# ToKe79/nuts333

Hardware: AMD Instinct MI355X
Metric: delivered_broadcast_lines_per_s (higher is better)
Workload: dtype u8

## Files before the change

### nuts333_amd/device/fanout.hip

```cpp

#include <hip/hip_runtime.h>
#include <hipcub/hipcub.hpp>

#include <algorithm>
#include <chrono>
#include <cstdint>
#include <cstdio>
#include <cstring>

namespace {

constexpr int kOutBuff = 1000;
constexpr int kTextSize = 2000;
constexpr int kNumCols = 21;
constexpr int kMaxWrites = 16;
constexpr int kBlock = 256;

constexpr uint8_t kLogin = 1, kHasRoom = 2, kSameRoom = 4, kIgnall = 8, kIgnshout = 16, kSender = 32, kColour = 64;
constexpr int kComShout = 4, kComSemote = 7;

__constant__ char kColCom[kNumCols][2] = {
    {'R', 'S'}, {'O', 'L'}, {'U', 'L'}, {'L', 'I'}, {'R', 'V'}, {'F', 'K'}, {'F', 'R'}, {'F', 'G'}, {'F', 'Y'}, {'F', 'B'},
    {'F', 'M'}, {'F', 'T'}, {'F', 'W'}, {'B', 'K'}, {'B', 'R'}, {'B', 'G'}, {'B', 'Y'}, {'B', 'B'}, {'B', 'M'}, {'B', 'T'},
    {'B', 'W'},
// ... 79 lines not shown
        } else if (ch == '~') {
            if (k.pos > kOutBuff - 6) k.flush();
            const int c = colcom_at(s, i, len);
            if (c >= 0) {
                if (colour) {
                    k.put(27); k.put('['); k.put((uint8_t)kColArg[c][0]);
                    if (kColArg[c][1]) k.put((uint8_t)kColArg[c][1]);
                    k.put('m');
                }
                i += 3;
            } else {
                k.put('~');
                i++;
            }
        } else {
            k.put(ch);
            i++;
        }
        if (k.pos == kOutBuff) k.flush();
    }
    if (k.pos) k.flush();
    if (colour) {
        k.reset_code();
        k.flush();
    }
}

struct Args {
    const uint8_t* text;
    const int32_t* text_off;
    const int32_t* text_len;
    const uint8_t* rec;
    int n;
    int rm_is_null, force_listen, com_num;
    uint8_t* admitted;
    int64_t* nbytes;
    int32_t* nwrites;
    int64_t* out_off;
    int32_t* w_off;
    int* violations;
    uint8_t* arena;
    int64_t arena_cap;
    int32_t* wsz;
    int64_t wsz_cap;
};

template <bool BROADCAST>
__device__ __forceinline__ bool load_item(const Args& a, int i, const uint8_t*& s, int& len)
{
    if (BROADCAST) {
        __shared__ uint8_t lds[kTextSize];
        len = a.text_len[0];
        for (int j = threadIdx.x; j < len; j += blockDim.x) lds[j] = a.text[j];
        __syncthreads();
        s = lds;
        return i < a.n;
    }
    if (i >= a.n) return false;
    s = a.text + a.text_off[i];
    len = a.text_len[i];
    return true;
}

template <bool BROADCAST>
__device__ void measure(const Args& a)
{
    const int i = blockIdx.x * blockDim.x + threadIdx.x;
    if (i == 0) {
        a.nbytes[a.n] = 0;
        a.nwrites[a.n] = 0;
    }
    const uint8_t* s;
    int len;
    if (!load_item<BROADCAST>(a, i, s, len)) return;
    const uint8_t l = a.rec[i];
    const bool in = !BROADCAST || admits(l, a.rm_is_null, a.force_listen, a.com_num);
    Sink<false> k{nullptr, nullptr, 0, 0};
    if (in) transduce(s, len, (l & kColour) != 0, k);
    if (k.n > 6 * (int64_t)len + 4 || k.writes > kMaxWrites) atomicAdd(a.violations, 1);
    a.admitted[i] = in;
    a.nbytes[i] = k.n;
    a.nwrites[i] = k.writes;
}

template <bool BROADCAST>
__device__ void emit(const Args& a)
{
    const int i = blockIdx.x * blockDim.x + threadIdx.x;
    const uint8_t* s;
    int len;
    if (!load_item<BROADCAST>(a, i, s, len) || !a.admitted[i]) return;
    const int64_t room = a.arena_cap - a.out_off[i], wroom = a.wsz_cap - a.w_off[i];
    const int64_t cap = a.nbytes[i] < room ? a.nbytes[i] : (room > 0 ? room : 0);
    const int wcap = (int)(a.nwrites[i] < wroom ? a.nwrites[i] : (wroom > 0 ? wroom : 0));
    Sink<true> k{a.arena + a.out_off[i], a.wsz + a.w_off[i], cap, wcap};
    transduce(s, len, (a.rec[i] & kColour) != 0, k);
}

constexpr int kVarCap = 6 * (kTextSize - 1) + 4;
constexpr int kGroup = 16;

struct ManyArgs {
    const uint8_t* text;
    const int32_t* text_off;
    const int32_t* text_len;
    const uint8_t* flags;
    const int32_t* com_num;
    const int32_t* item_off;
    const int32_t* tile_off;
    const uint8_t* rec;
    int k, m;
    int* violations;
    uint8_t* admitted;
    int64_t* out_off;
    int32_t* w_off;
    int64_t* nbytes;
    int32_t* nwrites;
    uint8_t* arena;
    int64_t arena_cap;
    int32_t* wsz;
    int64_t wsz_cap;
};

struct Tile {
    int b, lo, hi;
};

__device__ __forceinline__ Tile find_tile(const ManyArgs& a)
{
// ... 238 lines not shown
            const int64_t off = a.out_off[i], woff = a.w_off[i];
            const int64_t room = a.arena_cap - off, wroom = a.wsz_cap - woff;
            int64_t n = in ? a.out_off[i + 1] - off : 0;
            n = n < room ? n : room;
            n = n < cap ? n : cap;
            int64_t nw = in ? a.w_off[i + 1] - woff : 0;
            nw = nw < wroom ? nw : wroom;
            nw = nw < kMaxWrites ? nw : kMaxWrites;
            s_off[threadIdx.x] = off;
            s_n[threadIdx.x] = n > 0 ? n : 0;
            s_woff[threadIdx.x] = (int32_t)woff;
            s_nw[threadIdx.x] = nw > 0 ? (int32_t)nw : 0;
            s_c[threadIdx.x] = (a.slot[j] & kColour) ? 1 : 0;
        }
    }
    const uint8_t* src = a.var + var_at(a.text_off[b], b);
    const int64_t stride = var_stride(len);
    for (int c = 0; c < 2; c++) {
        const int64_t n = a.vn[2 * b + c] < cap ? a.vn[2 * b + c] : cap;
        for (int64_t q = threadIdx.x; q < n; q += kBlock) var[c * kVarCap + q] = src[c * stride + q];
        const int nw = a.vw[2 * b + c] < kMaxWrites ? a.vw[2 * b + c] : kMaxWrites;
        if ((int)threadIdx.x < nw) vwsz[c * kMaxWrites + threadIdx.x] = a.vwsz[(2 * b + c) * kMaxWrites + threadIdx.x];
        if (threadIdx.x == 0) {
            vn[c] = n;
            vw[c] = nw;
        }
    }
    __syncthreads();
    const int count = a.capacity - j0 < kBlock ? a.capacity - j0 : kBlock;
    copy_items(count, var, vwsz, vn, vw, s_off, s_n, s_woff, s_nw, s_c, a.arena, a.wsz);
}

static_assert(2 * kMaxWrites <= kBlock, "roster kernels move a broadcast's chunk sizes with one lane each");

struct PlanArgs {
    const int32_t* room;
    const uint8_t* slot;
    const uint8_t* text;
    const int32_t* text_off;
    const int32_t* text_len;
    const int32_t* rm;
    const int32_t* sender;
    const uint8_t* flags;
    const int32_t* com_num;
    int k, capacity, tiles;
    int words;
    int* violations;
    int64_t* vn;
    int32_t* vw;
    int32_t* vwsz;
    uint64_t* bits;
    uint8_t* var;
};

__device__ void roster_plan(const PlanArgs& a)
{
    const int b = (int)blockIdx.x / a.tiles, tile = (int)blockIdx.x - b * a.tiles;
    const int j = tile * kBlock + (int)threadIdx.x;
    bool in = false;
    if (j < a.capacity) {
        const int rm = a.rm[b];
        const uint8_t l = listener_record(a.room[j], a.slot[j], rm, a.sender[b], j);
        in = admits(l, rm < 0, (a.flags[b] >> 1) & 1, a.com_num[b]);
    }
    const uint64_t word = __ballot(in);
    const int w = j >> 6;
// ... 2954 lines not shown
static_assert(64 * kReadSlice >= kArrSize && kWordLen + 7 <= 64, "roster_set: the word masks cover the longest inpstr, a lane per byte of word[1]");

struct SetOrderArgs {
    const int32_t* slot;
    const int32_t* rid;
    const uint8_t* com;
    int k;
    int8_t* outcome;
    int32_t* clen;

    static constexpr int kKeys = 4, kTexts = kSetTexts, kDeferred = kSetDeferred, kMapWords = 3 * kOrderSlotWords;
    __device__ void load(int b, bool live, int (&key)[kKeys]) const
    {
        key[0] = live ? slot[b] : 0, key[1] = live ? rid[b] : 0, key[2] = live && clen[b] >= 0, key[3] = live && com[b] == kComTopic;
    }
    static __device__ bool hit(const int (&key)[kKeys], const uint32_t* slots)
    {
        return bit_of(slots, key[0]) || (key[2] && bit_of(slots + kOrderSlotWords, key[1])) ||
               (key[3] && bit_of(slots + 2 * kOrderSlotWords, key[1]));
    }
    static __device__ void touch(const int (&key)[kKeys], int outcome, uint32_t* slots)
    {
        if (outcome > kSetIgntellOff) return;
        set_bit(slots, key[0]);
        if (outcome == kSetIgnallOn || outcome == kSetIgnallOff || outcome == kSetColourOn || outcome == kSetColourOff)
            set_bit(slots + kOrderSlotWords, key[1]);
        if (outcome == kSetTopicSet) set_bit(slots + 2 * kOrderSlotWords, key[1]);
    }
    __device__ void also_void(int) const {}
};

}

extern "C" __global__ void __launch_bounds__(kBlock) nuts_fanout_measure_batch(Args a) { measure<false>(a); }
extern "C" __global__ void __launch_bounds__(kBlock) nuts_fanout_measure_broadcast(Args a) { measure<true>(a); }
extern "C" __global__ void __launch_bounds__(kBlock) nuts_fanout_emit_batch(Args a) { emit<false>(a); }
extern "C" __global__ void __launch_bounds__(kBlock) nuts_fanout_emit_broadcast(Args a) { emit<true>(a); }
extern "C" __global__ void __launch_bounds__(kBlock) nuts_fanout_measure_many(ManyArgs a) { measure_many(a); }
extern "C" __global__ void __launch_bounds__(kBlock) nuts_fanout_emit_many(ManyArgs a) { emit_many(a); }
extern "C" __global__ void __launch_bounds__(kBlock) nuts_roster_measure(RosterArgs a) { roster_measure(a); }
extern "C" __global__ void __launch_bounds__(kBlock) nuts_roster_emit(RosterArgs a) { roster_emit(a); }
extern "C" __global__ void __launch_bounds__(kBlock) nuts_roster_plan(PlanArgs a) { roster_plan(a); }
extern "C" __global__ void __launch_bounds__(kBlock) nuts_roster_record(RecordArgs a) { roster_record<kRevLines>(a); }
extern "C" __global__ void __launch_bounds__(kBlock) nuts_roster_review(ReviewArgs a) { roster_review<kRevLines>(a); }
extern "C" __global__ void __launch_bounds__(kBlock) nuts_roster_speak(SpeakArgs a) { roster_speak(a); }
extern "C" __global__ void __launch_bounds__(kBlock) nuts_roster_speak_plan(SpeakPlanArgs a) { roster_speak_plan(a); }
extern "C" __global__ void __launch_bounds__(kBlock) nuts_roster_parse(ParseArgs a) { roster_parse(a); }
extern "C" __global__ void __launch_bounds__(kBlock) nuts_roster_tell(TellArgs a) { roster_tell(a); }
extern "C" __global__ void __launch_bounds__(kBlock) nuts_roster_record_tell(RecordArgs a) { roster_record<kTellLines>(a); }
extern "C" __global__ void __launch_bounds__(kBlock) nuts_roster_revtell(ReviewArgs a) { roster_review<kTellLines>(a); }
extern "C" __global__ void __launch_bounds__(kBlock) nuts_roster_look(LookArgs a) { roster_look(a); }
extern "C" __global__ void __launch_bounds__(kBlock) nuts_roster_relay(RelayArgs a) { roster_relay(a); }
extern "C" __global__ void __launch_bounds__(kBlock) nuts_roster_who(WhoArgs a) { roster_who(a); }
extern "C" __global__ void __launch_bounds__(kBlock) nuts_roster_who_shown(WhoArgs a) { roster_who_shown(a); }
extern "C" __global__ void __launch_bounds__(kBlock) nuts_roster_rooms_count(RoomsArgs a) { roster_rooms_count(a); }
extern "C" __global__ void __launch_bounds__(kBlock) nuts_roster_rooms_lines(RoomsArgs a) { roster_rooms_lines(a); }
extern "C" __global__ void __launch_bounds__(kBlock) nuts_roster_go(GoArgs a) { roster_go(a); }
extern "C" __global__ void __launch_bounds__(kBlock) nuts_roster_go_order(GoOrderArgs a) { order_events(a); }
extern "C" __global__ void __launch_bounds__(kBlock) nuts_roster_access(AccessArgs a) { roster_access(a); }
extern "C" __global__ void __launch_bounds__(kBlock) nuts_roster_access_order(AccessOrderArgs a) { order_events(a); }
extern "C" __global__ void __launch_bounds__(kBlock) nuts_roster_clone(CloneArgs a) { roster_clone(a); }
extern "C" __global__ void __launch_bounds__(kBlock) nuts_roster_clone_order(CloneOrderArgs a) { order_events(a); }
extern "C" __global__ void __launch_bounds__(kBlock) nuts_roster_set(SetArgs a) { roster_set(a); }
extern "C" __global__ void __launch_bounds__(kBlock) nuts_roster_set_order(SetOrderArgs a) { order_events(a); }


namespace {

struct Buffers {
    uint8_t* d_block = nullptr;
// ... 128 lines not shown
    if (timing) {
        timing->kernels_us = (double)ms * 1e3;
        timing->end_to_end_us = (t1 - t0) * 1e-3;
    }
    return 0;
}

template <typename T>
int fill_timing(T* timing, double t0, double t1, size_t h2d_bytes, size_t d2h_bytes)
{
    if (fill_timing(timing, t0, t1)) return -1;
    if (timing) {
        timing->h2d_bytes = (int64_t)h2d_bytes;
        timing->d2h_bytes = (int64_t)d2h_bytes;
    }
    return 0;
}

int check_bounds(int violations, const char* what)
{
    if (!violations) return 0;
    snprintf(g_err, sizeof(g_err), "%d %s(s) exceeded the hard output bounds (6*len+4 bytes, %d writes)", violations,
             what, kMaxWrites);
    return -1;
}

int fetch_results(const uint8_t* d, size_t res_at, size_t res_bytes)
{
    ND_CHECK(hipEventRecord(g.ev1, g.stream));
    ND_CHECK(hipMemcpyAsync(gm.res, d + res_at, res_bytes, hipMemcpyDeviceToHost, g.stream));
    ND_CHECK(hipStreamSynchronize(g.stream));
    return 0;
}

size_t layout_many(uintptr_t base, size_t text_bytes, size_t scan_bytes, ManyArgs& a, uint8_t** scan)
{
    Carver take{base};
    const size_t k = (size_t)a.k, m = (size_t)a.m;
    take(a.text, text_bytes);
    take(a.text_off, k);
    take(a.text_len, k);
    take(a.flags, k);
    take(a.com_num, k);
    take(a.item_off, k + 1);
    take(a.tile_off, k + 1);
    take(a.rec, m);
    take(a.violations, 1);
    take(a.admitted, m);
    take(a.out_off, m + 1);
    take(a.w_off, m + 1);
    take(a.nbytes, m + 1);
    take(a.nwrites, m + 1);
    take(a.arena, (size_t)a.arena_cap);
    take(a.wsz, (size_t)a.wsz_cap);
    take(*scan, scan_bytes);
    return take.at;
}

constexpr int kMaxRosters = 64;
constexpr int kMaxCapacity = 65536;

enum KeptId { kKeptSpeech, kKeptAfk, kKeptRooms, kKeptUdesc, kKeptWho, kKeptClones, kKeptNames, kKeptGo, kKeptCount };
struct KeptTable {
    const char* what;
    uint8_t* d = nullptr;
};

struct Roster {
    bool live = false;
    bool resident = false;
    int capacity = 0;
    int64_t rooms = 0;
    uint8_t* d = nullptr;
    uint8_t* mirror = nullptr;
    size_t cap_d = 0, cap_mirror = 0;
    int review_rooms = 0;
    uint8_t* rings = nullptr;
    bool revtell = false;
    uint8_t* tell_rings = nullptr;
    int look_rooms = 0;
    int clones = 0;
    KeptTable kept[kKeptCount] = {{"speaker table"}, {"AFK messages"}, {"room table"}, {"user descriptions"},
                                  {"who table"}, {"clone records"}, {"room names"}, {"go table"}};
};
Roster g_rosters[kMaxRosters];

void take_clones(Carver& take, int clones, const int32_t*& owner, const int32_t*& room, const uint8_t*& hear)
{
// ... 778 lines not shown
    return rocprim::make_transform_iterator(rocprim::make_counting_iterator(0),
                                            ItemCount<int32_t>{a.admitted, a.slot, a.vw, a.capacity, m});
}

Roster* roster_at(int handle)
{
    if (handle < 0 || handle >= kMaxRosters || !g_rosters[handle].live) {
        snprintf(g_err, sizeof(g_err), "no live roster %d", handle);
        return nullptr;
    }
    return &g_rosters[handle];
}

}

extern "C" {

struct nd_timing {
    double kernels_us;
    double end_to_end_us;
};

const char* nd_last_error(void) { return g_err; }

int nd_device_count(void)
{
    int n = 0;
    hipError_t e = hipGetDeviceCount(&n);
    if (e == hipErrorNoDevice) return 0;
    if (e != hipSuccess) return fail("hipGetDeviceCount", e);
    return n;
}

int nd_fanout(int broadcast, const uint8_t* text, int64_t text_bytes, const int32_t* text_off, const int32_t* text_len,
              const uint8_t* rec, int n, int rm_is_null, int force_listen, int com_num, uint8_t* admitted,
              int64_t* out_off, int32_t* w_off, nd_timing* timing)
{
    if (ensure_ready()) return -1;
    if (n < 1) {
        snprintf(g_err, sizeof(g_err), "empty batch");
        return -1;
    }
    const double t0 = now_ns();
    hipStream_t st = g.stream;
    Args a{};
    a.n = n;
    a.rm_is_null = rm_is_null;
    a.force_listen = force_listen;
    a.com_num = com_num;
    a.arena_cap = 4 * (int64_t)n + 6 * text_bytes * (broadcast ? n : 1);
    a.wsz_cap = (int64_t)n * kMaxWrites;
    size_t scan1 = 0, scan2 = 0;
    ND_CHECK(hipcub::DeviceScan::ExclusiveSum(nullptr, scan1, a.nbytes, a.out_off, n + 1, st));
    ND_CHECK(hipcub::DeviceScan::ExclusiveSum(nullptr, scan2, a.nwrites, a.w_off, n + 1, st));
    const size_t scan_bytes = std::max(scan1, scan2);
    uint8_t* scan = nullptr;
    const size_t need = layout(0, (size_t)text_bytes, scan_bytes, a, &scan);
    if (grow_dev(&g.d_block, &g.cap_block, need, "device buffers")) return -1;
    layout((uintptr_t)g.d_block, (size_t)text_bytes, scan_bytes, a, &scan);

    ND_CHECK(hipMemcpyAsync((void*)a.text, text, (size_t)text_bytes, hipMemcpyHostToDevice, st));
    ND_CHECK(hipMemcpyAsync((void*)a.text_len, text_len, (broadcast ? 1 : (size_t)n) * sizeof(int32_t), hipMemcpyHostToDevice, st));
    if (!broadcast) ND_CHECK(hipMemcpyAsync((void*)a.text_off, text_off, (size_t)n * sizeof(int32_t), hipMemcpyHostToDevice, st));
    ND_CHECK(hipMemcpyAsync((void*)a.rec, rec, (size_t)n, hipMemcpyHostToDevice, st));
    ND_CHECK(hipMemsetAsync(a.violations, 0, sizeof(int), st));

    const dim3 grid((unsigned)((n + kBlock - 1) / kBlock)), block(kBlock);
    ND_CHECK(hipEventRecord(g.ev0, st));
    hipLaunchKernelGGL(broadcast ? nuts_fanout_measure_broadcast : nuts_fanout_measure_batch, grid, block, 0, st, a);
    ND_CHECK(hipGetLastError());
    size_t bytes = scan_bytes;
    ND_CHECK(hipcub::DeviceScan::ExclusiveSum(scan, bytes, a.nbytes, a.out_off, n + 1, st));
    bytes = scan_bytes;
    ND_CHECK(hipcub::DeviceScan::ExclusiveSum(scan, bytes, a.nwrites, a.w_off, n + 1, st));
    hipLaunchKernelGGL(broadcast ? nuts_fanout_emit_broadcast : nuts_fanout_emit_batch, grid, block, 0, st, a);
    ND_CHECK(hipGetLastError());
    ND_CHECK(hipEventRecord(g.ev1, st));

    int violations = 0;
    ND_CHECK(hipMemcpyAsync(admitted, a.admitted, (size_t)n, hipMemcpyDeviceToHost, st));
    ND_CHECK(hipMemcpyAsync(out_off, a.out_off, ((size_t)n + 1) * sizeof(int64_t), hipMemcpyDeviceToHost, st));
    ND_CHECK(hipMemcpyAsync(w_off, a.w_off, ((size_t)n + 1) * sizeof(int32_t), hipMemcpyDeviceToHost, st));
    ND_CHECK(hipMemcpyAsync(&violations, a.violations, sizeof(int), hipMemcpyDeviceToHost, st));
    ND_CHECK(hipStreamSynchronize(st));
    if (check_bounds(violations, "item")) return -1;
    if (grow_host(&g.h_arena, &g.cap_host_arena, (size_t)out_off[n] + 1, "pinned arena")) return -1;
    if (grow_host(&g.h_wsz, &g.cap_host_writes, (size_t)w_off[n] + 1, "pinned write sizes")) return -1;
    ND_CHECK(hipMemcpyAsync(g.h_arena, a.arena, (size_t)out_off[n], hipMemcpyDeviceToHost, st));
    ND_CHECK(hipMemcpyAsync(g.h_wsz, a.wsz, (size_t)w_off[n] * sizeof(int32_t), hipMemcpyDeviceToHost, st));
    ND_CHECK(hipStreamSynchronize(st));
    const double t1 = now_ns();

    return fill_timing(timing, t0, t1);
}

const uint8_t* nd_arena(void) { return g.h_arena; }
const int32_t* nd_write_sizes(void) { return g.h_wsz; }

int nd_fanout_many(int k, const uint8_t* text, int64_t text_bytes, const int32_t* text_off, const int32_t* text_len,
                   const uint8_t* flags, const int32_t* com_num, const int32_t* item_off, const uint8_t* rec,
                   uint8_t* admitted, int64_t* out_off, int32_t* w_off, nd_timing* timing)
{
    if (ensure_ready()) return -1;
    if (k < 1 || item_off[0] != 0) {
        snprintf(g_err, sizeof(g_err), "empty call, or item offsets that do not start at 0");
        return -1;
    }
    for (int b = 0; b < k; b++)
// ... 1327 lines not shown
```

### nuts333_amd/devpath.py

```python
from __future__ import annotations

import argparse
import ctypes
import json
import statistics
import subprocess
import sys
import time
from pathlib import Path
from typing import NamedTuple

import numpy as np

from nuts333_amd import device, nuts_path

REPO = Path(__file__).resolve().parent.parent
PATHBENCH = REPO / "oracle" / "_build" / "pathbench"

TEXTS = {
    "say": b"Uaaa says: synthetic broadcast line 000123 from the nuts333 bench\n",
    "shout": b"~OLUaaa shouts:~RS synthetic broadcast line 000123 from the nuts333 bench\n",
}
COM = {"say": device.COM_SAY, "shout": device.COM_SHOUT}
SIZES = (10, 100, 1000)
# ... 1140 lines not shown
    if ngpu < 1:
        print("devpath: no GPU visible; this command measures the device path and has no CPU fall-back",
              file=sys.stderr)
        return 2

    t_start = time.perf_counter()
    pb = pathbench(a.pathbench_iterations)
    cases = []
    for n in SIZES:
        for text in TEXTS:
            for colour in COLOURS:
                table = listeners(n, colour)
                run = lambda: device.broadcast(TEXTS[text], table, 0, 0, COM[text])
                first = run()
                expect = sum(len(nuts_path.transduce(TEXTS[text], int(c))) for c in colours(n, colour)[1:])
                if int(first.out_offsets[-1]) != expect or int(first.admitted.sum()) != n - 1:
                    raise SystemExit(f"devpath: {n}/{text}/{colour}: device produced {int(first.out_offsets[-1])} "
                                     f"bytes, the CPU restatement {expect}")
                times = _timed(f"{n}/{text}/{colour}", {"broadcast": run}, a.reps, a.warmup)["broadcast"].times
                cpu = cpu_derived_us(pb, text, colour, n)
                cases.append({"n": n, "text": text, "colour": colour, "recipients": n - 1,
                              "bytes_out": int(first.out_offsets[-1]), "writes": int(first.write_offsets[-1]),
                              "kernels_us": times["kernels_us"], "end_to_end_us": times["end_to_end_us"],
                              "cpu_derived_us": round(cpu, 3),
                              "end_to_end_over_cpu": round(times["end_to_end_us"]["median"] / cpu, 1)})
    sections = {}
    for option, _, _, section in SECTIONS:
        counts = getattr(a, option.replace("-", "_"))
        if counts:
            sections.update(globals()[section](counts, a.reps, a.warmup, pb))
    out = {
        "what": "user-space stage of one broadcast (admit predicate + transducer), device vs CPU",
        "device": "gfx950",
        "kernels": ["nuts_fanout_measure_broadcast", "rocprim device scan x2", "nuts_fanout_emit_broadcast"],
        "reps": a.reps, "warmup": a.warmup,
        "end_to_end_covers": "listener table + text H2D, kernels, admitted/offsets/arena/write-size D2H, synchronise",
        "cpu_derived_from": {"pathbench": {k: v for k, v in pb.items() if k not in ("sink", "admitted")},
                             "formula": "(N-1) x transduce + N x fanout_predicate + format_line_once (derived, not timed)"},
        "cases": cases,
        **sections,
        "wall_s": round(time.perf_counter() - t_start, 1),
    }
    print(json.dumps(out))
    return 0


if __name__ == "__main__":
    sys.exit(main())
```

Before: 738,300.

## Broadcast fanout: transduce two colour variants once, place recipients by tile counts

The broadcast path no longer transduces the text once per recipient and runs two device scans. Instead it renders the coloured and plain variants once, counts admitted recipients per colour in each tile with ballots, and computes every output offset arithmetically from those counts. It also packs all inputs into one pinned H2D copy and copies results back in a head-sized D2H with a tail copy only when needed. This removes per-recipient transducer work, the scan launches, and several small transfers and syncs. In exchange the emit kernel serially sums the counts of all earlier tiles and uses more LDS.

```diff
diff --git a/nuts333_amd/device/fanout.hip b/nuts333_amd/device/fanout.hip
--- a/nuts333_amd/device/fanout.hip
+++ b/nuts333_amd/device/fanout.hip
@@ -135,7 +135,6 @@
     const int32_t* text_len;
     const uint8_t* rec;
     int n;
-    int rm_is_null, force_listen, com_num;
     uint8_t* admitted;
     int64_t* nbytes;
     int32_t* nwrites;
@@ -148,24 +147,14 @@
     int64_t wsz_cap;
 };
 
-template <bool BROADCAST>
 __device__ __forceinline__ bool load_item(const Args& a, int i, const uint8_t*& s, int& len)
 {
-    if (BROADCAST) {
-        __shared__ uint8_t lds[kTextSize];
-        len = a.text_len[0];
-        for (int j = threadIdx.x; j < len; j += blockDim.x) lds[j] = a.text[j];
-        __syncthreads();
-        s = lds;
-        return i < a.n;
-    }
     if (i >= a.n) return false;
     s = a.text + a.text_off[i];
     len = a.text_len[i];
     return true;
 }
 
-template <bool BROADCAST>
 __device__ void measure(const Args& a)
 {
     const int i = blockIdx.x * blockDim.x + threadIdx.x;
@@ -175,24 +164,22 @@
     }
     const uint8_t* s;
     int len;
-    if (!load_item<BROADCAST>(a, i, s, len)) return;
+    if (!load_item(a, i, s, len)) return;
     const uint8_t l = a.rec[i];
-    const bool in = !BROADCAST || admits(l, a.rm_is_null, a.force_listen, a.com_num);
     Sink<false> k{nullptr, nullptr, 0, 0};
-    if (in) transduce(s, len, (l & kColour) != 0, k);
+    transduce(s, len, (l & kColour) != 0, k);
     if (k.n > 6 * (int64_t)len + 4 || k.writes > kMaxWrites) atomicAdd(a.violations, 1);
-    a.admitted[i] = in;
+    a.admitted[i] = true;
     a.nbytes[i] = k.n;
     a.nwrites[i] = k.writes;
 }
 
-template <bool BROADCAST>
 __device__ void emit(const Args& a)
 {
     const int i = blockIdx.x * blockDim.x + threadIdx.x;
     const uint8_t* s;
     int len;
-    if (!load_item<BROADCAST>(a, i, s, len) || !a.admitted[i]) return;
+    if (!load_item(a, i, s, len) || !a.admitted[i]) return;
     const int64_t room = a.arena_cap - a.out_off[i], wroom = a.wsz_cap - a.w_off[i];
     const int64_t cap = a.nbytes[i] < room ? a.nbytes[i] : (room > 0 ? room : 0);
     const int wcap = (int)(a.nwrites[i] < wroom ? a.nwrites[i] : (wroom > 0 ? wroom : 0));
@@ -502,6 +489,144 @@
 }
 
 static_assert(2 * kMaxWrites <= kBlock, "roster kernels move a broadcast's chunk sizes with one lane each");
+
+struct BroadcastArgs {
+    const uint8_t* text;
+    const int32_t* text_off;
+    const int32_t* text_len;
+    const uint8_t* rec;
+    int n;
+    int rm_is_null, force_listen, com_num;
+    int* violations;
+    uint8_t* admitted;
+    int32_t* tile_cnt;
+    int64_t* out_off;
+    int32_t* w_off;
+    uint8_t* var;
+    int64_t* vn;
+    int32_t* vw;
+    int32_t* vwsz;
+    uint8_t* arena;
+    int64_t arena_cap;
+    int32_t* wsz;
+    int64_t wsz_cap;
+};
+
+constexpr int kWaves = kBlock / 64;
+
+__device__ __forceinline__ void count_tile(bool in, int c, int (*cnt)[kWaves], uint64_t* below)
+{
+    const uint64_t b0 = __ballot(in && c == 0), b1 = __ballot(in && c != 0);
+    const int wave = (int)threadIdx.x >> 6, lane = (int)threadIdx.x & 63;
+    if (lane == 0) {
+        cnt[0][wave] = __popcll(b0);
+        cnt[1][wave] = __popcll(b1);
+    }
+    const uint64_t lt = ((uint64_t)1 << lane) - 1;
+    below[0] = b0 & lt;
+    below[1] = b1 & lt;
+    __syncthreads();
+}
+
+__device__ void broadcast_measure(const BroadcastArgs& a)
+{
+    __shared__ int cnt[2][kWaves];
+    const int64_t i = (int64_t)blockIdx.x * kBlock + threadIdx.x;
+    bool in = false;
+    int c = 0;
+    if (i < a.n) {
+        const uint8_t l = a.rec[i];
+        in = admits(l, a.rm_is_null, a.force_listen, a.com_num);
+        c = (l & kColour) ? 1 : 0;
+        a.admitted[i] = in;
+    }
+    uint64_t below[2];
+    count_tile(in, c, cnt, below);
+    if (threadIdx.x < 2) {
+        int sum = 0;
+        for (int w = 0; w < kWaves; w++) sum += cnt[threadIdx.x][w];
+        a.tile_cnt[2 * (int64_t)blockIdx.x + threadIdx.x] = sum;
+    }
+    if (blockIdx.x == 0) store_variants(a, 0);
+}
+
+__device__ void broadcast_emit(const BroadcastArgs& a)
+{
+    __shared__ uint8_t var[2 * kVarCap];
+    __shared__ int32_t vwsz[2 * kMaxWrites];
+    __shared__ int64_t vn[2];
+    __shared__ int vw[2];
+    __shared__ int64_t s_off[kBlock], s_n[kBlock];
+    __shared__ int32_t s_woff[kBlock], s_nw[kBlock];
+    __shared__ uint8_t s_c[kBlock];
+    __shared__ int cnt[2][kWaves];
+    __shared__ int base[2];
+    const int64_t i0 = (int64_t)blockIdx.x * kBlock, i = i0 + threadIdx.x;
+    const int len = a.text_len[0];
+    const int64_t cap = 6 * (int64_t)len + 4;
+    if (threadIdx.x < 2) base[threadIdx.x] = 0;
+    bool in = false;
+    int c = 0;
+    if (i < a.n) {
+        in = a.admitted[i] != 0;
+        c = (a.rec[i] & kColour) ? 1 : 0;
+    }
+    uint64_t below[2];
+    count_tile(in, c, cnt, below);
+    {
+        int t0 = 0, t1 = 0;
+        for (int t = (int)threadIdx.x; t < (int)blockIdx.x; t += kBlock) {
+            t0 += a.tile_cnt[2 * (int64_t)t];
+            t1 += a.tile_cnt[2 * (int64_t)t + 1];
+        }
+        if (t0) atomicAdd(&base[0], t0);
+        if (t1) atomicAdd(&base[1], t1);
+    }
+    const int64_t stride = var_stride(len);
+    for (int v = 0; v < 2; v++) {
+        const int64_t n = a.vn[v] < cap ? a.vn[v] : cap;
+        for (int64_t q = threadIdx.x; q < n; q += kBlock) var[v * kVarCap + q] = a.var[v * stride + q];
+        const int nw = a.vw[v] < kMaxWrites ? a.vw[v] : kMaxWrites;
+        if ((int)threadIdx.x < nw) vwsz[v * kMaxWrites + threadIdx.x] = a.vwsz[v * kMaxWrites + threadIdx.x];
+        if (threadIdx.x == 0) {
+            vn[v] = n;
+            vw[v] = nw;
+        }
+    }
+    __syncthreads();
+    if (i < a.n) {
+        const int wave = (int)threadIdx.x >> 6;
+        int64_t e0 = base[0] + __popcll(below[0]), e1 = base[1] + __popcll(below[1]);
+        for (int w = 0; w < wave; w++) {
+            e0 += cnt[0][w];
+            e1 += cnt[1][w];
+        }
+        const int64_t off = e0 * a.vn[0] + e1 * a.vn[1];
+        const int64_t woff = e0 * (int64_t)a.vw[0] + e1 * (int64_t)a.vw[1];
+        const int64_t mine = in ? a.vn[c] : 0, wmine = in ? a.vw[c] : 0;
+        a.out_off[i] = off;
+        a.w_off[i] = (int32_t)woff;
+        if (i == a.n - 1) {
+            a.out_off[a.n] = off + mine;
+            a.w_off[a.n] = (int32_t)(woff + wmine);
+        }
+        const int64_t room = a.arena_cap - off, wroom = a.wsz_cap - woff;
+        int64_t n = mine < room ? mine : room;
+        n = n < cap ? n : cap;
+        int64_t nw = wmine < wroom ? wmine : wroom;
+        nw = nw < kMaxWrites ? nw : kMaxWrites;
+        s_off[threadIdx.x] = off;
+        s_n[threadIdx.x] = n > 0 ? n : 0;
+        s_woff[threadIdx.x] = (int32_t)woff;
+        s_nw[threadIdx.x] = nw > 0 ? (int32_t)nw : 0;
+        s_c[threadIdx.x] = (uint8_t)c;
+    }
+    __syncthreads();
+    const int64_t left = a.n - i0;
+    copy_items(left < kBlock ? (int)left : kBlock, var, vwsz, vn, vw, s_off, s_n, s_woff, s_nw, s_c, a.arena, a.wsz);
+}
+
+static_assert(kWaves >= 1 && kBlock >= 2, "the broadcast kernels: whole waves, and a lane per colour");
 
 struct PlanArgs {
     const int32_t* room;
@@ -3522,10 +3647,10 @@
 
 }
 
-extern "C" __global__ void __launch_bounds__(kBlock) nuts_fanout_measure_batch(Args a) { measure<false>(a); }
-extern "C" __global__ void __launch_bounds__(kBlock) nuts_fanout_measure_broadcast(Args a) { measure<true>(a); }
-extern "C" __global__ void __launch_bounds__(kBlock) nuts_fanout_emit_batch(Args a) { emit<false>(a); }
-extern "C" __global__ void __launch_bounds__(kBlock) nuts_fanout_emit_broadcast(Args a) { emit<true>(a); }
+extern "C" __global__ void __launch_bounds__(kBlock) nuts_fanout_measure_batch(Args a) { measure(a); }
+extern "C" __global__ void __launch_bounds__(kBlock) nuts_fanout_measure_broadcast(BroadcastArgs a) { broadcast_measure(a); }
+extern "C" __global__ void __launch_bounds__(kBlock) nuts_fanout_emit_batch(Args a) { emit(a); }
+extern "C" __global__ void __launch_bounds__(kBlock) nuts_fanout_emit_broadcast(BroadcastArgs a) { broadcast_emit(a); }
 extern "C" __global__ void __launch_bounds__(kBlock) nuts_fanout_measure_many(ManyArgs a) { measure_many(a); }
 extern "C" __global__ void __launch_bounds__(kBlock) nuts_fanout_emit_many(ManyArgs a) { emit_many(a); }
 extern "C" __global__ void __launch_bounds__(kBlock) nuts_roster_measure(RosterArgs a) { roster_measure(a); }
@@ -3720,6 +3845,31 @@
     ND_CHECK(hipStreamSynchronize(g.stream));
     return 0;
 }
+
+size_t layout_broadcast(uintptr_t base, size_t text_bytes, BroadcastArgs& a)
+{
+    Carver take{base};
+    const size_t n = (size_t)a.n, tiles = (n + kBlock - 1) / kBlock;
+    take(a.text, text_bytes);
+    take(a.text_off, 1);
+    take(a.text_len, 1);
+    take(a.rec, n);
+    take(a.violations, 1);
+    take(a.vn, 2);
+    take(a.vw, 2);
+    take(a.admitted, n);
+    take(a.out_off, n + 1);
+    take(a.w_off, n + 1);
+    take(a.wsz, (size_t)a.wsz_cap);
+    take(a.arena, (size_t)a.arena_cap);
+    take(a.tile_cnt, 2 * tiles);
+    take(a.vwsz, 2 * kMaxWrites);
+    take(a.var, (size_t)(2 * var_stride((int)text_bytes)));
+    return take.at;
+}
+
+constexpr int64_t kArenaHeadPerItem = 128;
+constexpr int64_t kWszHeadPerItem = 4;
 
 size_t layout_many(uintptr_t base, size_t text_bytes, size_t scan_bytes, ManyArgs& a, uint8_t** scan)
 {
@@ -4586,6 +4736,100 @@
     return n;
 }
 
+void nd_fanout_heads(int n, int64_t* arena_head_bytes, int64_t* wsz_head_entries)
+{
+    *arena_head_bytes = (int64_t)n * kArenaHeadPerItem;
+    *wsz_head_entries = (int64_t)n * kWszHeadPerItem;
+}
+
+static int fanout_broadcast(const uint8_t* text, int64_t text_bytes, int len, const uint8_t* rec, int n, int rm_is_null, int force_listen,
+                            int com_num, uint8_t* admitted, int64_t* out_off, int32_t* w_off, nd_timing* timing)
+{
+    if (len < 0 || len >= kTextSize || len > text_bytes) {
+        snprintf(g_err, sizeof(g_err), "a text of %d bytes: need 0 .. %d, and no more than were given", len, kTextSize - 1);
+        return -1;
+    }
+    const double t0 = now_ns();
+    hipStream_t st = g.stream;
+    BroadcastArgs a{};
+    a.n = n;
+    a.rm_is_null = rm_is_null;
+    a.force_listen = force_listen;
+    a.com_num = com_num;
+    a.arena_cap = (int64_t)n * (6 * (int64_t)len + 4);
+    a.wsz_cap = (int64_t)n * kMaxWrites;
+    BroadcastArgs o = a;
+    const size_t need = layout_broadcast(0, (size_t)len, o);
+    if (grow_dev(&g.d_block, &g.cap_block, need, "device buffers")) return -1;
+    layout_broadcast((uintptr_t)g.d_block, (size_t)len, a);
+    int64_t arena_head = 0, wsz_head = 0;
+    nd_fanout_heads(n, &arena_head, &wsz_head);
+    arena_head = std::min(arena_head, a.arena_cap);
+    wsz_head = std::min(wsz_head, a.wsz_cap);
+    const size_t in_bytes = (uintptr_t)o.violations + sizeof(int);
+    const size_t res_at = (uintptr_t)o.violations;
+    const size_t res_bytes = (uintptr_t)o.wsz + (size_t)wsz_head * sizeof(int32_t) - res_at;
+    if (grow_host(&gm.stage, &gm.cap_stage, in_bytes, "pinned staging")) return -1;
+    if (grow_host(&gm.res, &gm.cap_res, res_bytes, "pinned results")) return -1;
+    if (grow_host(&g.h_arena, &g.cap_host_arena, (size_t)arena_head + 1, "pinned arena")) return -1;
+    if (grow_host(&g.h_wsz, &g.cap_host_writes, (size_t)wsz_head + 1, "pinned write sizes")) return -1;
+
+    uint8_t* h = gm.stage;
+    const Put put{h};
+    put(o.text, text, (size_t)len);
+    *reinterpret_cast<int32_t*>(h + (uintptr_t)o.text_off) = 0;
+    *reinterpret_cast<int32_t*>(h + (uintptr_t)o.text_len) = len;
+    put(o.rec, rec, (size_t)n);
+    *reinterpret_cast<int*>(h + (uintptr_t)o.violations) = 0;
+    ND_CHECK(hipMemcpyAsync(g.d_block, h, in_bytes, hipMemcpyHostToDevice, st));
+
+    const dim3 grid((unsigned)((n + kBlock - 1) / kBlock)), block(kBlock);
+    ND_CHECK(hipEventRecord(g.ev0, st));
+    hipLaunchKernelGGL(nuts_fanout_measure_broadcast, grid, block, 0, st, a);
+    ND_CHECK(hipGetLastError());
+    hipLaunchKernelGGL(nuts_fanout_emit_broadcast, grid, block, 0, st, a);
+    ND_CHECK(hipGetLastError());
+    ND_CHECK(hipEventRecord(g.ev1, st));
+
+    ND_CHECK(hipMemcpyAsync(gm.res, g.d_block + res_at, res_bytes, hipMemcpyDeviceToHost, st));
+    if (arena_head) ND_CHECK(hipMemcpyAsync(g.h_arena, a.arena, (size_t)arena_head, hipMemcpyDeviceToHost, st));
+    ND_CHECK(hipStreamSynchronize(st));
+    const Res res{gm.res, res_at};
+    if (check_bounds(*reinterpret_cast<const int*>(res(o.violations)), "variant")) return -1;
+    memcpy(admitted, res(o.admitted), (size_t)n);
+    memcpy(out_off, res(o.out_off), ((size_t)n + 1) * sizeof(int64_t));
+    memcpy(w_off, res(o.w_off), ((size_t)n + 1) * sizeof(int32_t));
+
+    const int64_t total = out_off[n], wtotal = w_off[n];
+    bool tail = false;
+    if (wtotal > wsz_head) {
+        int64_t from = wsz_head;
+        if ((size_t)wtotal + 1 > g.cap_host_writes) {
+            if (grow_host(&g.h_wsz, &g.cap_host_writes, (size_t)wtotal + 1, "pinned write sizes")) return -1;
+            from = 0;
+        }
+        memcpy(g.h_wsz, res(o.wsz), (size_t)from * sizeof(int32_t));
+        ND_CHECK(hipMemcpyAsync(g.h_wsz + from, a.wsz + from, (size_t)(wtotal - from) * sizeof(int32_t),
+                                hipMemcpyDeviceToHost, st));
+        tail = true;
+    } else if (wtotal > 0) {
+        memcpy(g.h_wsz, res(o.wsz), (size_t)wtotal * sizeof(int32_t));
+    }
+    if (total > arena_head) {
+        int64_t from = arena_head;
+        if ((size_t)total + 1 > g.cap_host_arena) {
+            if (grow_host(&g.h_arena, &g.cap_host_arena, (size_t)total + 1, "pinned arena")) return -1;
+            from = 0;
+        }
+        ND_CHECK(hipMemcpyAsync(g.h_arena + from, a.arena + from, (size_t)(total - from), hipMemcpyDeviceToHost, st));
+        tail = true;
+    }
+    if (tail) ND_CHECK(hipStreamSynchronize(st));
+    const double t1 = now_ns();
+
+    return fill_timing(timing, t0, t1);
+}
+
 int nd_fanout(int broadcast, const uint8_t* text, int64_t text_bytes, const int32_t* text_off, const int32_t* text_len,
               const uint8_t* rec, int n, int rm_is_null, int force_listen, int com_num, uint8_t* admitted,
               int64_t* out_off, int32_t* w_off, nd_timing* timing)
@@ -4595,14 +4839,14 @@
         snprintf(g_err, sizeof(g_err), "empty batch");
         return -1;
     }
+    if (broadcast)
+        return fanout_broadcast(text, text_bytes, text_len[0], rec, n, rm_is_null, force_listen, com_num, admitted, out_off, w_off,
+                                timing);
     const double t0 = now_ns();
     hipStream_t st = g.stream;
     Args a{};
     a.n = n;
-    a.rm_is_null = rm_is_null;
-    a.force_listen = force_listen;
-    a.com_num = com_num;
-    a.arena_cap = 4 * (int64_t)n + 6 * text_bytes * (broadcast ? n : 1);
+    a.arena_cap = 4 * (int64_t)n + 6 * text_bytes;
     a.wsz_cap = (int64_t)n * kMaxWrites;
     size_t scan1 = 0, scan2 = 0;
     ND_CHECK(hipcub::DeviceScan::ExclusiveSum(nullptr, scan1, a.nbytes, a.out_off, n + 1, st));
@@ -4614,20 +4858,20 @@
     layout((uintptr_t)g.d_block, (size_t)text_bytes, scan_bytes, a, &scan);
 
     ND_CHECK(hipMemcpyAsync((void*)a.text, text, (size_t)text_bytes, hipMemcpyHostToDevice, st));
-    ND_CHECK(hipMemcpyAsync((void*)a.text_len, text_len, (broadcast ? 1 : (size_t)n) * sizeof(int32_t), hipMemcpyHostToDevice, st));
-    if (!broadcast) ND_CHECK(hipMemcpyAsync((void*)a.text_off, text_off, (size_t)n * sizeof(int32_t), hipMemcpyHostToDevice, st));
+    ND_CHECK(hipMemcpyAsync((void*)a.text_len, text_len, (size_t)n * sizeof(int32_t), hipMemcpyHostToDevice, st));
+    ND_CHECK(hipMemcpyAsync((void*)a.text_off, text_off, (size_t)n * sizeof(int32_t), hipMemcpyHostToDevice, st));
     ND_CHECK(hipMemcpyAsync((void*)a.rec, rec, (size_t)n, hipMemcpyHostToDevice, st));
     ND_CHECK(hipMemsetAsync(a.violations, 0, sizeof(int), st));
 
     const dim3 grid((unsigned)((n + kBlock - 1) / kBlock)), block(kBlock);
     ND_CHECK(hipEventRecord(g.ev0, st));
-    hipLaunchKernelGGL(broadcast ? nuts_fanout_measure_broadcast : nuts_fanout_measure_batch, grid, block, 0, st, a);
+    hipLaunchKernelGGL(nuts_fanout_measure_batch, grid, block, 0, st, a);
     ND_CHECK(hipGetLastError());
     size_t bytes = scan_bytes;
     ND_CHECK(hipcub::DeviceScan::ExclusiveSum(scan, bytes, a.nbytes, a.out_off, n + 1, st));
     bytes = scan_bytes;
     ND_CHECK(hipcub::DeviceScan::ExclusiveSum(scan, bytes, a.nwrites, a.w_off, n + 1, st));
-    hipLaunchKernelGGL(broadcast ? nuts_fanout_emit_broadcast : nuts_fanout_emit_batch, grid, block, 0, st, a);
+    hipLaunchKernelGGL(nuts_fanout_emit_batch, grid, block, 0, st, a);
     ND_CHECK(hipGetLastError());
     ND_CHECK(hipEventRecord(g.ev1, st));
 
diff --git a/nuts333_amd/devpath.py b/nuts333_amd/devpath.py
--- a/nuts333_amd/devpath.py
+++ b/nuts333_amd/devpath.py
@@ -1196,9 +1196,11 @@
     out = {
         "what": "user-space stage of one broadcast (admit predicate + transducer), device vs CPU",
         "device": "gfx950",
-        "kernels": ["nuts_fanout_measure_broadcast", "rocprim device scan x2", "nuts_fanout_emit_broadcast"],
+        "kernels": ["nuts_fanout_measure_broadcast", "nuts_fanout_emit_broadcast"],
         "reps": a.reps, "warmup": a.warmup,
-        "end_to_end_covers": "listener table + text H2D, kernels, admitted/offsets/arena/write-size D2H, synchronise",
+        "end_to_end_covers": "packing the listener table and the text into pinned memory, one H2D, two kernels, two D2H "
+                             "(admitted, offsets and write sizes; the arena) at sizes the listeners decide, one "
+                             "synchronise; an output past those sizes adds a D2H of the rest and a synchronise",
         "cpu_derived_from": {"pathbench": {k: v for k, v in pb.items() if k not in ("sink", "admitted")},
                              "formula": "(N-1) x transduce + N x fanout_predicate + format_line_once (derived, not timed)"},
         "cases": cases,
```

New measurement: 731,200. About the same (-1.0%).

## Transduce broadcast text once per colour variant and replicate instead of per recipient

Applied to the files above, without the earlier changes.

The broadcast path used to run the transducer for every recipient, then two device scans, then a second transduction in emit. Now one block precomputes the two colour variants (plain and colour) and the measure kernel only evaluates admission. The emit kernel derives each recipient's offset in closed form from counts of admitted plain and colour recipients via ballots, and copies the cached variant bytes. Host staging is packed into a single H2D and results are fetched in one block. This removes redundant per-recipient transduction and the scan launches. In exchange, every block rescans all earlier admitted flags, which is quadratic in recipient count.

```diff
diff --git a/nuts333_amd/device/fanout.hip b/nuts333_amd/device/fanout.hip
--- a/nuts333_amd/device/fanout.hip
+++ b/nuts333_amd/device/fanout.hip
@@ -135,7 +135,6 @@
     const int32_t* text_len;
     const uint8_t* rec;
     int n;
-    int rm_is_null, force_listen, com_num;
     uint8_t* admitted;
     int64_t* nbytes;
     int32_t* nwrites;
@@ -148,24 +147,6 @@
     int64_t wsz_cap;
 };
 
-template <bool BROADCAST>
-__device__ __forceinline__ bool load_item(const Args& a, int i, const uint8_t*& s, int& len)
-{
-    if (BROADCAST) {
-        __shared__ uint8_t lds[kTextSize];
-        len = a.text_len[0];
-        for (int j = threadIdx.x; j < len; j += blockDim.x) lds[j] = a.text[j];
-        __syncthreads();
-        s = lds;
-        return i < a.n;
-    }
-    if (i >= a.n) return false;
-    s = a.text + a.text_off[i];
-    len = a.text_len[i];
-    return true;
-}
-
-template <bool BROADCAST>
 __device__ void measure(const Args& a)
 {
     const int i = blockIdx.x * blockDim.x + threadIdx.x;
@@ -173,31 +154,25 @@
         a.nbytes[a.n] = 0;
         a.nwrites[a.n] = 0;
     }
-    const uint8_t* s;
-    int len;
-    if (!load_item<BROADCAST>(a, i, s, len)) return;
-    const uint8_t l = a.rec[i];
-    const bool in = !BROADCAST || admits(l, a.rm_is_null, a.force_listen, a.com_num);
+    if (i >= a.n) return;
+    const int len = a.text_len[i];
     Sink<false> k{nullptr, nullptr, 0, 0};
-    if (in) transduce(s, len, (l & kColour) != 0, k);
+    transduce(a.text + a.text_off[i], len, (a.rec[i] & kColour) != 0, k);
     if (k.n > 6 * (int64_t)len + 4 || k.writes > kMaxWrites) atomicAdd(a.violations, 1);
-    a.admitted[i] = in;
+    a.admitted[i] = 1;
     a.nbytes[i] = k.n;
     a.nwrites[i] = k.writes;
 }
 
-template <bool BROADCAST>
 __device__ void emit(const Args& a)
 {
     const int i = blockIdx.x * blockDim.x + threadIdx.x;
-    const uint8_t* s;
-    int len;
-    if (!load_item<BROADCAST>(a, i, s, len) || !a.admitted[i]) return;
+    if (i >= a.n) return;
     const int64_t room = a.arena_cap - a.out_off[i], wroom = a.wsz_cap - a.w_off[i];
     const int64_t cap = a.nbytes[i] < room ? a.nbytes[i] : (room > 0 ? room : 0);
     const int wcap = (int)(a.nwrites[i] < wroom ? a.nwrites[i] : (wroom > 0 ? wroom : 0));
     Sink<true> k{a.arena + a.out_off[i], a.wsz + a.w_off[i], cap, wcap};
-    transduce(s, len, (a.rec[i] & kColour) != 0, k);
+    transduce(a.text + a.text_off[i], a.text_len[i], (a.rec[i] & kColour) != 0, k);
 }
 
 constexpr int kVarCap = 6 * (kTextSize - 1) + 4;
@@ -502,6 +477,114 @@
 }
 
 static_assert(2 * kMaxWrites <= kBlock, "roster kernels move a broadcast's chunk sizes with one lane each");
+
+struct SingleArgs {
+    const uint8_t* text;
+    const int32_t* text_off;
+    const int32_t* text_len;
+    const uint8_t* rec;
+    int n;
+    int rm_is_null, force_listen, com_num;
+    int* violations;
+    uint8_t* admitted;
+    int64_t* out_off;
+    int32_t* w_off;
+    uint8_t* var;
+    int64_t* vn;
+    int32_t* vw;
+    int32_t* vwsz;
+    uint8_t* arena;
+    int64_t arena_cap;
+    int32_t* wsz;
+    int64_t wsz_cap;
+};
+
+__device__ void single_measure(const SingleArgs& a)
+{
+    const int i = (int)blockIdx.x * kBlock + (int)threadIdx.x;
+    if (i < a.n) a.admitted[i] = admits(a.rec[i], a.rm_is_null, a.force_listen, a.com_num);
+    if (blockIdx.x == 0) store_variants(a, 0);
+}
+
+__device__ void single_emit(const SingleArgs& a)
+{
+    __shared__ uint8_t var[2 * kVarCap];
+    __shared__ int32_t vwsz[2 * kMaxWrites];
+    __shared__ int64_t vn[2];
+    __shared__ int vw[2];
+    __shared__ int64_t s_off[kBlock], s_n[kBlock];
+    __shared__ int32_t s_woff[kBlock], s_nw[kBlock];
+    __shared__ uint8_t s_c[kBlock];
+    __shared__ int s_before[kBlock / 64][2];
+    __shared__ int s_tile[kBlock / 64][2];
+    const int j0 = (int)blockIdx.x * kBlock;
+    const int len = a.text_len[0];
+    const int64_t cap = 6 * (int64_t)len + 4;
+    const int64_t stride = var_stride(len);
+    for (int c = 0; c < 2; c++) {
+        const int64_t n = a.vn[c] < cap ? a.vn[c] : cap;
+        for (int64_t q = threadIdx.x; q < n; q += kBlock) var[c * kVarCap + q] = a.var[c * stride + q];
+        const int nw = a.vw[c] < kMaxWrites ? a.vw[c] : kMaxWrites;
+        if ((int)threadIdx.x < nw) vwsz[c * kMaxWrites + threadIdx.x] = a.vwsz[c * kMaxWrites + threadIdx.x];
+        if (threadIdx.x == 0) {
+            vn[c] = n;
+            vw[c] = nw;
+        }
+    }
+    int c0 = 0, c1 = 0;
+    for (int q = (int)threadIdx.x; q < j0; q += kBlock)
+        if (a.admitted[q]) {
+            if (a.rec[q] & kColour) c1++;
+            else c0++;
+        }
+    for (int d = 32; d > 0; d >>= 1) {
+        c0 += __shfl_down(c0, d);
+        c1 += __shfl_down(c1, d);
+    }
+    const int i = j0 + (int)threadIdx.x;
+    const int lane = (int)threadIdx.x & 63, wave = (int)threadIdx.x >> 6;
+    const bool in = i < a.n && a.admitted[i] != 0;
+    const bool on = i < a.n && (a.rec[i] & kColour) != 0;
+    const uint64_t b0 = __ballot(in && !on), b1 = __ballot(in && on);
+    if (lane == 0) {
+        s_before[wave][0] = c0;
+        s_before[wave][1] = c1;
+        s_tile[wave][0] = __popcll(b0);
+        s_tile[wave][1] = __popcll(b1);
+    }
+    __syncthreads();
+    if (i < a.n) {
+        const uint64_t below = (1ull << lane) - 1;
+        int64_t a0 = __popcll(b0 & below), a1 = __popcll(b1 & below);
+        for (int w = 0; w < kBlock / 64; w++) {
+            a0 += s_before[w][0] + (w < wave ? s_tile[w][0] : 0);
+            a1 += s_before[w][1] + (w < wave ? s_tile[w][1] : 0);
+        }
+        const int64_t off = a0 * a.vn[0] + a1 * a.vn[1], woff = a0 * a.vw[0] + a1 * a.vw[1];
+        const int64_t size = in ? a.vn[on] : 0, writes = in ? a.vw[on] : 0;
+        a.out_off[i] = off;
+        a.w_off[i] = (int32_t)woff;
+        if (i == a.n - 1) {
+            a.out_off[a.n] = off + size;
+            a.w_off[a.n] = (int32_t)(woff + writes);
+        }
+        const int64_t room = a.arena_cap - off, wroom = a.wsz_cap - woff;
+        int64_t n = size < room ? size : room;
+        n = n < cap ? n : cap;
+        int64_t nw = writes < wroom ? writes : wroom;
+        nw = nw < kMaxWrites ? nw : kMaxWrites;
+        s_off[threadIdx.x] = off;
+        s_n[threadIdx.x] = n > 0 ? n : 0;
+        s_woff[threadIdx.x] = (int32_t)woff;
+        s_nw[threadIdx.x] = nw > 0 ? (int32_t)nw : 0;
+        s_c[threadIdx.x] = on ? 1 : 0;
+    }
+    __syncthreads();
+    const int count = a.n - j0 < kBlock ? a.n - j0 : kBlock;
+    copy_items(count, var, vwsz, vn, vw, s_off, s_n, s_woff, s_nw, s_c, a.arena, a.wsz);
+}
+
+static_assert(kBlock % 64 == 0, "single_emit: a tile is whole waves, two ballots each");
 
 struct PlanArgs {
     const int32_t* room;
@@ -3522,10 +3605,10 @@
 
 }
 
-extern "C" __global__ void __launch_bounds__(kBlock) nuts_fanout_measure_batch(Args a) { measure<false>(a); }
-extern "C" __global__ void __launch_bounds__(kBlock) nuts_fanout_measure_broadcast(Args a) { measure<true>(a); }
-extern "C" __global__ void __launch_bounds__(kBlock) nuts_fanout_emit_batch(Args a) { emit<false>(a); }
-extern "C" __global__ void __launch_bounds__(kBlock) nuts_fanout_emit_broadcast(Args a) { emit<true>(a); }
+extern "C" __global__ void __launch_bounds__(kBlock) nuts_fanout_measure_batch(Args a) { measure(a); }
+extern "C" __global__ void __launch_bounds__(kBlock) nuts_fanout_measure_broadcast(SingleArgs a) { single_measure(a); }
+extern "C" __global__ void __launch_bounds__(kBlock) nuts_fanout_emit_batch(Args a) { emit(a); }
+extern "C" __global__ void __launch_bounds__(kBlock) nuts_fanout_emit_broadcast(SingleArgs a) { single_emit(a); }
 extern "C" __global__ void __launch_bounds__(kBlock) nuts_fanout_measure_many(ManyArgs a) { measure_many(a); }
 extern "C" __global__ void __launch_bounds__(kBlock) nuts_fanout_emit_many(ManyArgs a) { emit_many(a); }
 extern "C" __global__ void __launch_bounds__(kBlock) nuts_roster_measure(RosterArgs a) { roster_measure(a); }
@@ -3742,6 +3825,27 @@
     take(a.arena, (size_t)a.arena_cap);
     take(a.wsz, (size_t)a.wsz_cap);
     take(*scan, scan_bytes);
+    return take.at;
+}
+
+size_t layout_single(uintptr_t base, size_t text_bytes, SingleArgs& a)
+{
+    Carver take{base};
+    const size_t n = (size_t)a.n;
+    take(a.text, text_bytes);
+    take(a.text_off, 1);
+    take(a.text_len, 1);
+    take(a.rec, n);
+    take(a.violations, 1);
+    take(a.admitted, n);
+    take(a.out_off, n + 1);
+    take(a.w_off, n + 1);
+    take(a.var, (size_t)var_at((int64_t)text_bytes, 1));
+    take(a.vn, 2);
+    take(a.vw, 2);
+    take(a.vwsz, 2 * kMaxWrites);
+    take(a.arena, (size_t)a.arena_cap);
+    take(a.wsz, (size_t)a.wsz_cap);
     return take.at;
 }
 
@@ -4595,14 +4699,63 @@
         snprintf(g_err, sizeof(g_err), "empty batch");
         return -1;
     }
+    if (broadcast && text_len[0] != text_bytes) {
+        snprintf(g_err, sizeof(g_err), "a broadcast's text_len[0] must be its text_bytes");
+        return -1;
+    }
     const double t0 = now_ns();
     hipStream_t st = g.stream;
+    if (broadcast) {
+        SingleArgs a{};
+        a.n = n;
+        a.rm_is_null = rm_is_null;
+        a.force_listen = force_listen;
+        a.com_num = com_num;
+        a.arena_cap = (int64_t)n * (6 * text_bytes + 4);
+        a.wsz_cap = (int64_t)n * kMaxWrites;
+        SingleArgs o = a;
+        const size_t need = layout_single(0, (size_t)text_bytes, o);
+        if (grow_dev(&g.d_block, &g.cap_block, need, "device buffers")) return -1;
+        layout_single((uintptr_t)g.d_block, (size_t)text_bytes, a);
+        const size_t in_bytes = (uintptr_t)o.violations + sizeof(int);
+        const size_t res_at = (uintptr_t)o.violations, res_bytes = (uintptr_t)o.var - res_at;
+        if (grow_host(&gm.stage, &gm.cap_stage, in_bytes, "pinned staging")) return -1;
+        if (grow_host(&gm.res, &gm.cap_res, res_bytes, "pinned results")) return -1;
+
+        uint8_t* h = gm.stage;
+        const Put put{h};
+        const int32_t zero = 0;
+        put(o.text, text, (size_t)text_bytes);
+        put(o.text_off, &zero, sizeof(int32_t));
+        put(o.text_len, text_len, sizeof(int32_t));
+        put(o.rec, rec, (size_t)n);
+        put(o.violations, &zero, sizeof(int));
+        ND_CHECK(hipMemcpyAsync(g.d_block, h, in_bytes, hipMemcpyHostToDevice, st));
+
+        const dim3 grid((unsigned)((n + kBlock - 1) / kBlock)), block(kBlock);
+        ND_CHECK(hipEventRecord(g.ev0, st));
+        hipLaunchKernelGGL(nuts_fanout_measure_broadcast, grid, block, 0, st, a);
+        ND_CHECK(hipGetLastError());
+        hipLaunchKernelGGL(nuts_fanout_emit_broadcast, grid, block, 0, st, a);
+        ND_CHECK(hipGetLastError());
+
+        if (fetch_results(g.d_block, res_at, res_bytes)) return -1;
+        const Res res{gm.res, res_at};
+        if (check_bounds(*reinterpret_cast<const int*>(res(o.violations)), "variant")) return -1;
+        memcpy(admitted, res(o.admitted), (size_t)n);
+        memcpy(out_off, res(o.out_off), ((size_t)n + 1) * sizeof(int64_t));
+        memcpy(w_off, res(o.w_off), ((size_t)n + 1) * sizeof(int32_t));
+        if (grow_host(&g.h_arena, &g.cap_host_arena, (size_t)out_off[n] + 1, "pinned arena")) return -1;
+        if (grow_host(&g.h_wsz, &g.cap_host_writes, (size_t)w_off[n] + 1, "pinned write sizes")) return -1;
+        ND_CHECK(hipMemcpyAsync(g.h_arena, a.arena, (size_t)out_off[n], hipMemcpyDeviceToHost, st));
+        ND_CHECK(hipMemcpyAsync(g.h_wsz, a.wsz, (size_t)w_off[n] * sizeof(int32_t), hipMemcpyDeviceToHost, st));
+        ND_CHECK(hipStreamSynchronize(st));
+        const double t1 = now_ns();
+        return fill_timing(timing, t0, t1);
+    }
     Args a{};
     a.n = n;
-    a.rm_is_null = rm_is_null;
-    a.force_listen = force_listen;
-    a.com_num = com_num;
-    a.arena_cap = 4 * (int64_t)n + 6 * text_bytes * (broadcast ? n : 1);
+    a.arena_cap = 4 * (int64_t)n + 6 * text_bytes;
     a.wsz_cap = (int64_t)n * kMaxWrites;
     size_t scan1 = 0, scan2 = 0;
     ND_CHECK(hipcub::DeviceScan::ExclusiveSum(nullptr, scan1, a.nbytes, a.out_off, n + 1, st));
@@ -4614,20 +4767,20 @@
     layout((uintptr_t)g.d_block, (size_t)text_bytes, scan_bytes, a, &scan);
 
     ND_CHECK(hipMemcpyAsync((void*)a.text, text, (size_t)text_bytes, hipMemcpyHostToDevice, st));
-    ND_CHECK(hipMemcpyAsync((void*)a.text_len, text_len, (broadcast ? 1 : (size_t)n) * sizeof(int32_t), hipMemcpyHostToDevice, st));
-    if (!broadcast) ND_CHECK(hipMemcpyAsync((void*)a.text_off, text_off, (size_t)n * sizeof(int32_t), hipMemcpyHostToDevice, st));
+    ND_CHECK(hipMemcpyAsync((void*)a.text_len, text_len, (size_t)n * sizeof(int32_t), hipMemcpyHostToDevice, st));
+    ND_CHECK(hipMemcpyAsync((void*)a.text_off, text_off, (size_t)n * sizeof(int32_t), hipMemcpyHostToDevice, st));
     ND_CHECK(hipMemcpyAsync((void*)a.rec, rec, (size_t)n, hipMemcpyHostToDevice, st));
     ND_CHECK(hipMemsetAsync(a.violations, 0, sizeof(int), st));
 
     const dim3 grid((unsigned)((n + kBlock - 1) / kBlock)), block(kBlock);
     ND_CHECK(hipEventRecord(g.ev0, st));
-    hipLaunchKernelGGL(broadcast ? nuts_fanout_measure_broadcast : nuts_fanout_measure_batch, grid, block, 0, st, a);
+    hipLaunchKernelGGL(nuts_fanout_measure_batch, grid, block, 0, st, a);
     ND_CHECK(hipGetLastError());
     size_t bytes = scan_bytes;
     ND_CHECK(hipcub::DeviceScan::ExclusiveSum(scan, bytes, a.nbytes, a.out_off, n + 1, st));
     bytes = scan_bytes;
     ND_CHECK(hipcub::DeviceScan::ExclusiveSum(scan, bytes, a.nwrites, a.w_off, n + 1, st));
-    hipLaunchKernelGGL(broadcast ? nuts_fanout_emit_broadcast : nuts_fanout_emit_batch, grid, block, 0, st, a);
+    hipLaunchKernelGGL(nuts_fanout_emit_batch, grid, block, 0, st, a);
     ND_CHECK(hipGetLastError());
     ND_CHECK(hipEventRecord(g.ev1, st));
 
diff --git a/nuts333_amd/devpath.py b/nuts333_amd/devpath.py
--- a/nuts333_amd/devpath.py
+++ b/nuts333_amd/devpath.py
@@ -1196,9 +1196,10 @@
     out = {
         "what": "user-space stage of one broadcast (admit predicate + transducer), device vs CPU",
         "device": "gfx950",
-        "kernels": ["nuts_fanout_measure_broadcast", "rocprim device scan x2", "nuts_fanout_emit_broadcast"],
+        "kernels": ["nuts_fanout_measure_broadcast", "nuts_fanout_emit_broadcast"],
         "reps": a.reps, "warmup": a.warmup,
-        "end_to_end_covers": "listener table + text H2D, kernels, admitted/offsets/arena/write-size D2H, synchronise",
+        "end_to_end_covers": "packing the listener table and the text into pinned memory, one H2D, two kernels, three D2H "
+                             "(admitted and the offsets; the arena; the write sizes), two synchronises",
         "cpu_derived_from": {"pathbench": {k: v for k, v in pb.items() if k not in ("sink", "admitted")},
                              "formula": "(N-1) x transduce + N x fanout_predicate + format_line_once (derived, not timed)"},
         "cases": cases,
```

Result: no change. 733,300 before, 729,400 after (-0.5%).
